# ChenAnno/FashionERN_AAAI2024

Hardware: AMD Instinct MI355X
Metric: composed queries/sec (higher is better)
Workload: dtype f32; 1 GPU; FashionIQ ViT-B/16 composed queries: 64-query batch per GPU vs 46k-image fused gallery (BASELINE.json configs[1]); clip=ViT-B-16, query_batch_per_gpu=64, gallery_rows=46000, gallery_dtype=f32, feature_dim=512, top_k=50, batches_in_flight=4, hw_queues=4, parallelism=dp1 queries

## Files before the change

### fashionern_aaai2024_amd/csrc/api.hip

```cpp
#include <hip/hip_runtime.h>

#include <algorithm>
#include <cmath>
#include <cstdio>
#include <cstdlib>
#include <cstring>
#include <map>
#include <string>
#include <vector>

#include "../../include/fern.h"
#include "kernels.h"
#include "live.h"

using namespace fern;

static thread_local std::string g_last_error;

static int fail(int code, const std::string& msg) {
    g_last_error = msg;
    return code;
}
#define HIP_TRY(expr)                                                                                   \
    do {                                                                                                \
// ... 310 lines not shown
    FERN_TRY(prof_open(c, PROF_GEMM, 2.0 * p1.M * (double)p1.N * p1.K + 2.0 * p2.M * (double)p2.N * p2.K, s, &slot, p1.M, p1.N, p1.K, 350 + p1.epi));
    const hipError_t le = launch_gemm_mxbf_pair(p1, p2, s);
    HIP_TRY_PROF(le, c, slot);
    if (slot >= 0) {
        c->recs[slot].dispatches = gemm_last_dispatches();
        c->recs[slot].extra_flops = 2.0 * p2.M * (double)p2.N * p2.K;
    }
    return prof_close(c, slot, s);
}
static int run_attention(fern_ctx* c, const AttnParams& a, hipStream_t s) {
    int slot;
    FERN_TRY(prof_open(c, PROF_ATTN, 4.0 * a.batch * a.heads * (double)a.s_q * a.s_k * a.hd, s, &slot, a.batch * a.heads, a.s_q, a.hd, a.causal));
    const hipError_t le = launch_attention(a, s);
    HIP_TRY_PROF(le, c, slot);
    return prof_close(c, slot, s);
}

static int make_bf16(fern_ctx* c, LinearW* L);

static int upload(fern_ctx* c, const float* h, size_t n, const float** out) {
    float* d = nullptr;
    HIP_TRY(hipMalloc(&d, std::max<size_t>(n, 4) * sizeof(float)));
    HIP_TRY(hipMemcpy(d, h, n * sizeof(float), hipMemcpyHostToDevice));
    c->owned[c->cur_group].push_back(d);
    *out = d;
    return FERN_OK;
}
static int need(fern_ctx* c, const std::string& key, std::vector<int64_t> shape, const HostTensor** out) {
    auto it = c->host.find(key);
    if (it == c->host.end()) return fail(FERN_ERR_STATE, "missing weight: " + key);
// ... 808 lines not shown
    const fern_clip_config& cf = W.cfg;
    const int g = cf.image_size / cf.patch_size;
    if (text) *T = Tower{W.tblocks.data(), batch, cf.context_length, cf.t_width, cf.t_heads, cf.t_mlp, 1};
    else *T = Tower{W.vblocks.data(), batch, g * g + 1, cf.v_width, cf.v_heads, cf.v_mlp, 0};
    tower_forms(c, text, T);
    const size_t R = (size_t)T->R();
    FERN_TRY(ws_get(c, R * T->width, &T->X));
    FERN_TRY(ws_get(c, R * T->width, &T->XN));
    FERN_TRY(ws_get(c, R * 3 * T->width, &T->QKV));
    FERN_TRY(ws_get(c, R * T->width, &T->ATT));
    return ws_get(c, R * T->mlp, &T->H);
}

static int run_gemm_form(fern_ctx* c, Form f, const GemmParams& p, hipStream_t s) { return f == F32 ? run_gemm(c, p, s) : run_gemm_b(c, p, s); }

static int ln_gemm(const Tower& T, Form f, const LNW& ln, const LinearW& L, void* C, long ldc, int epi, bool out_bf16, hipStream_t s, GemmParams* p) {
    const long R = T.R();
    const int w = T.width;
    switch (f) {
    case F32:
        HIP_TRY(launch_layernorm(T.X, nullptr, ln.g, ln.b, T.XN, R, w, w, w, 1e-5f, s));
        *p = gemm_desc(T.XN, w, L, reinterpret_cast<float*>(C), ldc, (int)R, epi);
        break;
    case BF16:
        HIP_TRY(launch_layernorm_bf16(T.X, ln.g, ln.b, T.XNb(), R, w, w, w, 1e-5f, s));
        *p = gemm_desc_b(T.XNb(), w, L, C, ldc, (int)R, epi, out_bf16);
        break;
    case FP8:
        HIP_TRY(launch_layernorm_fp8(T.X, ln.g, ln.b, T.XN8(), T.SA(), R, w, w, w, 1e-5f, s));
        *p = gemm_desc_f8(T.XN8(), T.SA(), w, L, C, ldc, (int)R, epi, out_bf16);
        break;
    case MX:
        HIP_TRY(launch_layernorm_mx8(T.Xb ? nullptr : T.X, ln.g, ln.b, T.XN8(), T.SM(), R, R, w, w, w, 1e-5f, s, T.Xb));
        *p = gemm_desc_mx(T.XN8(), T.SM(), R, w, L, C, ldc, (int)R, epi, out_bf16);
        break;
    }
    return FERN_OK;
}
static void residual_in_place(const Tower& T, GemmParams* p) {
    if (T.Xb) p->Rb = T.Xb;
    else p->R = T.X;
}

static int prep_qkv(fern_ctx*, const Tower& T, const ClipBlockW& Bk, hipStream_t s, GemmParams* p) {
    return ln_gemm(T, T.attn, Bk.ln1, Bk.qkv, T.QKV, 3 * T.width, EPI_BIAS, true, s, p);
}
static int prep_out(fern_ctx* c, const Tower& T, const ClipBlockW& Bk, hipStream_t s, GemmParams* p) {
    const long R = T.R();
    const int w = T.width, hd = w / T.heads;
    const bool fused = T.attn == MX && hd % 32 == 0;
    if (T.attn == F32) {
        AttnParams a{T.QKV, T.QKV + w, T.QKV + 2 * w, T.ATT, 3L * w, 3L * w, 3L * w, (long)w,
                     T.batch, T.heads, hd, T.S, T.S, T.causal, 1.0f / std::sqrt((float)hd)};
        FERN_TRY(run_attention(c, a, s));
    } else {
        AttnParams a{nullptr, nullptr, nullptr, nullptr, 3L * w, 3L * w, 3L * w, (long)w,
                     T.batch, T.heads, hd, T.S, T.S, T.causal, 1.0f / std::sqrt((float)hd), T.ATTb(), T.QKVb(), T.QKVb() + w, T.QKVb() + 2 * w};
        if (fused) { a.out_b = nullptr; a.out_q8 = T.ATT8(); a.out_scales = T.SM(); a.out_srows = R; }
        FERN_TRY(run_attention(c, a, s));
    }
    switch (T.attn) {
    case F32: *p = gemm_desc(T.ATT, w, Bk.out, T.X, w, (int)R, EPI_BIAS_RESIDUAL); break;
    case BF16: *p = gemm_desc_b(T.ATTb(), w, Bk.out, T.X, w, (int)R, EPI_BIAS_RESIDUAL, false); break;
    case FP8:
        HIP_TRY(launch_quantize_rows_fp8(T.ATTb(), nullptr, w, T.ATT8(), w, T.SA(), R, w, s));
        *p = gemm_desc_f8(T.ATT8(), T.SA(), w, Bk.out, T.X, w, (int)R, EPI_BIAS_RESIDUAL, false);
        break;
    case MX:
        if (!fused) HIP_TRY(launch_quantize_mx8(T.ATTb(), nullptr, w, T.ATT8(), w, T.SM(), R, R, w, s));
        *p = gemm_desc_mx(T.ATT8(), T.SM(), R, w, Bk.out, T.stream(), w, (int)R, EPI_BIAS_RESIDUAL, T.Xb != nullptr);
        break;
    }
    residual_in_place(T, p);
    return FERN_OK;
}
static int prep_fc(fern_ctx* c, const Tower& T, const ClipBlockW& Bk, hipStream_t s, GemmParams* p) {
    FERN_TRY(ln_gemm(T, T.mlpf, Bk.ln2, Bk.fc, T.H, T.mlp, clip_mlp_epi(c), T.mlpf != MX, s, p));
    if (T.mlpf == MX) { p->out_mx8 = 1; p->mxc = T.SH(); p->mxc_rows = T.R(); }
    return FERN_OK;
}
static int prep_proj(fern_ctx*, const Tower& T, const ClipBlockW& Bk, hipStream_t s, GemmParams* p) {
    const long R = T.R();
    const int w = T.width, mlp = T.mlp;
    switch (T.mlpf) {
    case F32: *p = gemm_desc(T.H, mlp, Bk.proj, T.X, w, (int)R, EPI_BIAS_RESIDUAL); break;
    case BF16: *p = gemm_desc_b(T.Hb(), mlp, Bk.proj, T.X, w, (int)R, EPI_BIAS_RESIDUAL, false); break;
    case FP8:
        HIP_TRY(launch_quantize_rows_fp8(T.Hb(), nullptr, mlp, T.H8(FP8), mlp, T.SA(), R, mlp, s));
        *p = gemm_desc_f8(T.H8(FP8), T.SA(), mlp, Bk.proj, T.X, w, (int)R, EPI_BIAS_RESIDUAL, false);
        break;
    case MX:
        *p = gemm_desc_mx(T.H8(MX), T.SH(), R, mlp, Bk.proj, T.stream(), w, (int)R, EPI_BIAS_RESIDUAL, T.Xb != nullptr);
        break;
// ... 271 lines not shown
    const fern_clip_config& cf = W.cfg;
    Tower V, T;
    float* CLS;
    int* eot;
    FERN_TRY(tower_open(c, false, b, &V));
    FERN_TRY(ws_get(c, (size_t)b * V.width, &CLS));
    FERN_TRY(tower_open(c, true, b, &T));
    FERN_TRY(ws_get(c, (size_t)b, &eot));
    FERN_TRY(vit_front(c, images, V.X, V.H, b, s));
    HIP_TRY(launch_layernorm(V.X, nullptr, W.ln_pre.g, W.ln_pre.b, V.X, V.R(), V.width, V.width, V.width, 1e-5f, s));
    HIP_TRY(launch_text_embed(tokens, W.tok_emb, W.tpos, T.X, eot, b, T.S, T.width, cf.vocab_size, c->tok_flag, s));
    const int vfull = cf.v_layers - 1;
    const int paired = vfull < cf.t_layers ? vfull : cf.t_layers;
    const bool mx = V.attn == MX;
    auto run_pair = [&](const GemmParams& pv, const GemmParams& pt) { return mx ? run_gemm_b_pair(c, pv, pt, s) : run_gemm_pair(c, pv, pt, s); };
    for (int l = 0; l < paired; ++l) {
        const ClipBlockW &Bv = V.blocks[l], &Bt = T.blocks[l];
        GemmParams pv, pt;
        FERN_TRY(prep_qkv(c, V, Bv, s, &pv));
        FERN_TRY(prep_qkv(c, T, Bt, s, &pt));
        FERN_TRY(run_pair(pv, pt));
        FERN_TRY(prep_out(c, V, Bv, s, &pv));
        FERN_TRY(prep_out(c, T, Bt, s, &pt));
        FERN_TRY(run_pair(pv, pt));
        FERN_TRY(prep_fc(c, V, Bv, s, &pv));
        FERN_TRY(prep_fc(c, T, Bt, s, &pt));
        FERN_TRY(run_pair(pv, pt));
        FERN_TRY(prep_proj(c, V, Bv, s, &pv));
        FERN_TRY(prep_proj(c, T, Bt, s, &pt));
        FERN_TRY(run_pair(pv, pt));
    }
    for (int l = paired; l < vfull; ++l) FERN_TRY(tower_block(c, V, l, s));
    for (int l = paired; l < cf.t_layers; ++l) FERN_TRY(tower_block(c, T, l, s));
    FERN_TRY(vit_tail(c, V, CLS, out_img, s));
    return text_tail(c, T.X, T.XN, eot, out_global, out_seq, b, s);
}

static int check_token_flag(fern_ctx* c, const char* fn) {
    if (!c->tok_flag) return FERN_OK;
    const int v = __atomic_load_n(c->tok_flag, __ATOMIC_RELAXED);
    if (v == 0) return FERN_OK;
    __atomic_store_n(c->tok_flag, 0, __ATOMIC_RELAXED);
// ... 1129 lines not shown
```

### fashionern_aaai2024_amd/csrc/attn.hip

```cpp
#include "kernels.h"

#include <cstdlib>

namespace fern {

typedef float f32x16 __attribute__((ext_vector_type(16)));
typedef float f32x4 __attribute__((ext_vector_type(4)));
typedef short bf16x8 __attribute__((ext_vector_type(8)));
typedef short s16x4 __attribute__((ext_vector_type(4)));
typedef unsigned u32x4_t __attribute__((ext_vector_type(4)));

extern __shared__ __attribute__((aligned(16))) char attn_smem[];

struct LanePos { int l31, lh, tr_off; };
__device__ __forceinline__ LanePos lane_pos() {
    const int lane = threadIdx.x & 63, lh = lane >> 5;
    return {lane & 31, lh, ((lane & 15) >> 2) * 64 + (((lane >> 4) & 1) * 16 + (lane & 3) * 4) * 2 + lh * 4 * 64};
}

template <int HDP_>
struct F32Form {
    static constexpr int HDP = HDP_;
    static constexpr bool BF16 = false;
    static constexpr int KS = HDP + 4;
// ... 246 lines not shown
__device__ __forceinline__ void store_out(const f32x16 (&o)[F::HDP / 32], float inv, int b, int h, int qi, int lh, const AttnParams& p) {
    if constexpr (!F::BF16) store_f32(o, inv, b, h, qi, lh, p);
    else if (p.out_q8) store_mx(o, inv, b, h, qi, lh, p);
    else store_bf16(o, inv, b, h, qi, lh, p);
}

template <int NB>
__device__ __forceinline__ void zero_acc(f32x16 (&o)[NB]) {
#pragma unroll
    for (int db = 0; db < NB; ++db)
#pragma unroll
        for (int r = 0; r < 16; ++r) o[db][r] = 0.0f;
}

template <class F, int NT, bool CAUSAL, int NW>
__device__ __forceinline__ void resident_walk(const AttnParams& p) {
    constexpr int ROWS = NT * 32;
    const int wave = threadIdx.x >> 6;
    const int b = blockIdx.x / p.heads, h = blockIdx.x % p.heads;
    F::template stage<ROWS>(p, b, h, 0, ROWS, threadIdx.x, NW * 64);
    __syncthreads();
    const LanePos lp = lane_pos();

    const int nqt = (p.s_q + 31) / 32;
    for (int qt = wave; qt < nqt; qt += NW) {
        const int qi = qt * 32 + lp.l31;
        typename F::Q qf;
        F::load_q(qf, p, b, h, qi < p.s_q ? qi : p.s_q - 1, lp.lh, true);
        f32x16 o[F::HDP / 32];
        zero_acc(o);
        float m = -INFINITY, sum = 0.0f;
        const int nt = CAUSAL ? (qt + 1 < NT ? qt + 1 : NT) : NT;
#pragma unroll 1
        for (int t = 0; t < nt; ++t) F::template key_tile<CAUSAL, ROWS>(t, t, qi, lp, p, qf, m, sum, o);
// ... 22 lines not shown
        const int nt = nkt - t0 < CT ? nkt - t0 : CT;
        if (t0) __syncthreads();
        F::template stage<ROWS>(p, b, h, t0 * 32, whole_image ? ROWS : nt * 32, threadIdx.x, stride);
        __syncthreads();
        if (!active) continue;
#pragma unroll 1
        for (int t = 0; t < nt; ++t) F::template key_tile<false, ROWS>(t, t0 + t, qi, lp, p, qf, m, sum, o);
    }
    if (!active) return;
    sum += __shfl_xor(sum, 32);
    store_out<F>(o, 1.0f / sum, b, h, qi, lp.lh, p);
}

template <int HDP, int NT, bool CAUSAL, int NW>
__global__ __launch_bounds__(NW * 64) void attn_f32_kernel(AttnParams p) {
    resident_walk<F32Form<HDP>, NT, CAUSAL, NW>(p);
}

template <int HDP, int NT, bool CAUSAL, int NW>
__global__ __launch_bounds__(NW * 64) void attn_bf16_kernel(AttnParams p) {
    resident_walk<Bf16Form<HDP>, NT, CAUSAL, NW>(p);
}

template <int HDP, int NT, int NW, int KH>
__global__ __launch_bounds__(NW * 64, 2) void attn_f32_chunked_kernel(AttnParams p) {
    chunk_walk<F32Form<HDP>, (NT + KH - 1) / KH>(p, StreamGroup{(int)blockIdx.x, 0, (p.s_q + 31) / 32}, NT, NW * 64, true);
}

constexpr int STREAM_CT = 4;
constexpr int STREAM_MAX_WAVES = 8;

__device__ __forceinline__ StreamGroup stream_group(int s_q) {
    const int nqt = (s_q + 31) / 32, ng = (nqt + STREAM_MAX_WAVES - 1) / STREAM_MAX_WAVES;
    const int base = nqt / ng, rem = nqt % ng, grp = blockIdx.x % ng;
    return {(int)(blockIdx.x / ng), grp * base + (grp < rem ? grp : rem), base + (grp < rem ? 1 : 0)};
}

template <int HDP>
__global__ __launch_bounds__(STREAM_MAX_WAVES * 64, HDP <= 64 ? 4 : 2) void attn_f32_stream_kernel(AttnParams p) {
    chunk_walk<F32Form<HDP>, STREAM_CT>(p, stream_group(p.s_q), (p.s_k + 31) / 32, blockDim.x, false);
}

template <int HDP>
__global__ __launch_bounds__(STREAM_MAX_WAVES * 64, 4) void attn_bf16_stream_kernel(AttnParams p) {
    chunk_walk<Bf16Form<HDP>, STREAM_CT>(p, stream_group(p.s_q), (p.s_k + 31) / 32, blockDim.x, false);
}

template <auto Kern>
static hipError_t launch_kernel(const AttnParams& p, dim3 grid, dim3 block, size_t lds, hipStream_t s) {
    static bool attr_set = false;
    if (!attr_set && lds > 48 * 1024) {
        hipError_t e = hipFuncSetAttribute(reinterpret_cast<const void*>(Kern), hipFuncAttributeMaxDynamicSharedMemorySize, (int)lds);
        if (e != hipSuccess) return e;
        attr_set = true;
    }
    FERN_LAUNCH(Kern, grid, block, lds, s, p);
    return hipGetLastError();
}

template <class F, int NT, bool CAUSAL>
// ... 102 lines not shown
        for (int u = 0; u < UNR; ++u) {
            const int j = j0 + 4 * u;
            vv[u] = vb[(long)(j < p.s_k ? j : p.s_k - 1) * p.ldv];
        }
#pragma unroll
        for (int u = 0; u < UNR; ++u) {
            const int j = j0 + 4 * u;
            acc = __builtin_fmaf(j < p.s_k ? sc[j] : 0.0f, vv[u], acc);
        }
    }
    red[wave][lane] = acc;
    __syncthreads();
    if (wave == 0 && lane < hd)
        p.out[(long)b * p.ldo + (long)h * hd + lane] = (((red[0][lane] + red[1][lane]) + red[2][lane]) + red[3][lane]) * (1.0f / sum);
}
hipError_t launch_attention(const AttnParams& p, hipStream_t s) {
    if (p.batch <= 0 || p.heads <= 0 || p.s_q <= 0 || p.s_k <= 0 || p.s_k > ATTN_MAX_KEYS) return hipErrorInvalidValue;
    if (p.causal && p.s_q != p.s_k) return hipErrorInvalidValue;
    if (p.qb || p.kb || p.vb) {
        if (!p.qb || !p.kb || !p.vb || (!p.out_b && !p.out_q8) || (p.out_q8 && (!p.out_scales || (p.hd & 31))) || (p.hd & 7) || (p.ldq & 7) || (p.ldk & 7) || (p.ldv & 7) || (p.ldo & 3)) return hipErrorInvalidValue;
        return launch_hd<Bf16Form>(p, s);
    }
    if (p.out_b || p.out_q8) return hipErrorInvalidValue;
    if ((p.hd & 3) || (p.ldq & 3) || (p.ldk & 3) || (p.ldv & 3) || (p.ldo & 3)) return hipErrorInvalidValue;
    if (p.s_q == 1 && !p.causal && p.hd <= 64 && p.s_k <= SQ1_MAX_KEYS) {
        FERN_LAUNCH(attn_f32_single_query_kernel<25>, dim3(p.batch * p.heads), dim3(256), 0, s, p);
        return hipGetLastError();
    }
    return launch_hd<F32Form>(p, s);
}

}
```

### fashionern_aaai2024_amd/csrc/elem.hip

```cpp
#include "kernels.h"
#include "row_ops.h"
#include <type_traits>

namespace fern {

__device__ __forceinline__ float wave_max(float v) {
    v = fmaxf(v, dpp_move<0xB1>(v));
    v = fmaxf(v, dpp_move<0x4E>(v));
    v = fmaxf(v, dpp_move<0x141>(v));
    v = fmaxf(v, dpp_move<0x140>(v));
    return fmaxf(fmaxf(lane_f(v, 0), lane_f(v, 16)), fmaxf(lane_f(v, 32), lane_f(v, 48)));
}
__device__ __forceinline__ float quad_max(float v) {
    v = fmaxf(v, dpp_move<0xB1>(v));
    return fmaxf(v, dpp_move<0x4E>(v));
}
__device__ __forceinline__ float oct_max(float v) { v = quad_max(v); return fmaxf(v, dpp_move<0x141>(v)); }

template <class V>
constexpr int chunk_width = sizeof(V) / sizeof(float);

__device__ __forceinline__ void load8(float (&v)[8], const float* p) {
    const f32x4 a = load4(p), b = load4(p + 4);
#pragma unroll
// ... 128 lines not shown
            if ((i * 64 + lane) * 4 < d) am = chunk_amax(am, r.v[i]);
        row_store_fp8(r.v, am, y + row * ldy, scale + row, d, lane);
    }
};
struct RowToMx8 {
    unsigned char* y; long ldy; unsigned char* scales; long srows;
    __device__ void operator()(const RowRegs& r, long row, int d, int lane) const {
#pragma unroll
        for (int i = 0; i < MAXV; ++i) {
            const int c = (i * 64 + lane) * 4;
            store_mx8(r.v[i], c < d, y + row * ldy, c, scales, srows, row, lane);
        }
    }
};
template <class T, class Out>
__global__ __launch_bounds__(256) void layernorm_kernel(const T* x, const float* gamma, const float* beta, Out out, long rows, int d, long ldx,
                                                        float eps, const float* res) {
    const long row = (long)blockIdx.x * ROWS_PER_BLOCK + (threadIdx.x >> 6);
    const int lane = threadIdx.x & 63;
    if (row >= rows) return;
    RowRegs r;
    row_load(r, x + row * ldx, d, lane);
    if constexpr (std::is_same_v<Out, RowToF32>) {
        if (res) {
            RowRegs q;
            row_load(q, res + row * ldx, d, lane);
#pragma unroll
            for (int i = 0; i < MAXV; ++i) r.v[i] += q.v[i];
        }
    }
    row_layernorm(r, gamma, beta, d, lane, eps);
    out(r, row, d, lane);
}

__device__ __forceinline__ void row_load8(float (&v)[8], const unsigned short* xb, const float* xf, long at, bool live) {
#pragma unroll
    for (int e = 0; e < 8; ++e) v[e] = 0.f;
    if (live) {
        if (xb) load8(v, xb + at);
        else load8(v, xf + at);
    }
}
__global__ __launch_bounds__(256) void quantize_rows_fp8_kernel(const unsigned short* xb, const float* xf, long ldx, unsigned char* y, long ldy,
                                                                float* scale, long rows, int d) {
    const long row = (long)blockIdx.x * ROWS_PER_BLOCK + (threadIdx.x >> 6);
    const int lane = threadIdx.x & 63;
    if (row >= rows) return;
    float v[8][8];
// ... 19 lines not shown
        store_mx8(v, c < d, y + row * ldy, c, scales, srows, row, lane);
    }
}

template <class F>
static void with_nv(int d, F f) {
    switch (d / 256) {
        case 1: f(std::integral_constant<int, 1>{}); break;
        case 2: f(std::integral_constant<int, 2>{}); break;
        case 3: f(std::integral_constant<int, 3>{}); break;
        default: f(std::integral_constant<int, 4>{}); break;
    }
}

template <int NV, int RPW>
__global__ __launch_bounds__(256) void layernorm_rows_kernel(const float* x, const float* gamma, const float* beta, float* y, long rows, long ldx,
                                                             long ldy, float eps) {
    constexpr int D = 256 * NV;
    const int lane = threadIdx.x & 63;
    const long row0 = ((long)blockIdx.x * ROWS_PER_BLOCK + (threadIdx.x >> 6)) * RPW;
    if (row0 >= rows) return;
    f32x4 v[RPW][NV];
#pragma unroll
    for (int r = 0; r < RPW; ++r) {
        const long row = row0 + r < rows ? row0 + r : rows - 1;
#pragma unroll
        for (int i = 0; i < NV; ++i) v[r][i] = load4(x + row * ldx + (i * 64 + lane) * 4);
    }
    f32x4 g[NV], bb[NV];
#pragma unroll
    for (int i = 0; i < NV; ++i) {
        g[i] = load4(gamma + (i * 64 + lane) * 4);
        bb[i] = load4(beta + (i * 64 + lane) * 4);
    }
    float mean[RPW], rstd[RPW];
// ... 8 lines not shown
            for (int e = 0; e < 4; ++e) { const float t = v[r][i][e] - mean[r]; q += t * t; }
        rstd[r] = rsqrtf(wave_sum(q) / (float)D + eps);
    }
#pragma unroll
    for (int r = 0; r < RPW; ++r) {
        const long row = row0 + r;
#pragma unroll
        for (int i = 0; i < NV; ++i) {
            f32x4 o;
#pragma unroll
            for (int e = 0; e < 4; ++e) o[e] = ln_affine(v[r][i][e], mean[r], rstd[r], g[i][e], bb[i][e]);
            if (row < rows) *reinterpret_cast<f32x4*>(y + row * ldy + (i * 64 + lane) * 4) = o;
        }
    }
}
constexpr int LN_RPW = 4;
static bool launch_ln_rows(const float* x, const float* gamma, const float* beta, float* y, long rows, int d, long ldx, long ldy, float eps,
                           hipStream_t s) {
    if (d % 256 || d > 1024) return false;
    if (((uintptr_t)gamma & 15) || ((uintptr_t)beta & 15)) return false;
    const dim3 grid((unsigned)((rows + ROWS_PER_BLOCK * LN_RPW - 1) / (ROWS_PER_BLOCK * LN_RPW)));
    with_nv(d, [&](auto nv) {
        hipLaunchKernelGGL((layernorm_rows_kernel<decltype(nv)::value, LN_RPW>), grid, dim3(256), 0, s, x, gamma, beta, y, rows, ldx, ldy, eps);
    });
    return true;
}

template <int NV, class T>
__global__ __launch_bounds__(256) void layernorm_half_kernel(const T* x, const float* gamma, const float* beta, unsigned char* y, unsigned char* scales,
                                                             long srows, long rows, long ldx, long ldy, float eps) {
    constexpr int D = 256 * NV;
    const int lane = threadIdx.x & 63, l31 = lane & 31, lh = lane >> 5;
    const long rowp = ((long)blockIdx.x * ROWS_PER_BLOCK + (threadIdx.x >> 6)) * 2;
    if (rowp >= rows) return;
    const long row = rowp + lh;
    const long rrow = row < rows ? row : rows - 1;
    float v[NV][8], g[NV][8], bb[NV][8];
#pragma unroll
    for (int i = 0; i < NV; ++i) load8(v[i], x + rrow * ldx + (i * 32 + l31) * 8);
#pragma unroll
    for (int i = 0; i < NV; ++i) {
        load8(g[i], gamma + (i * 32 + l31) * 8);
        load8(bb[i], beta + (i * 32 + l31) * 8);
    }
    const auto half_sum = [&](float t) {
        t += dpp_move<0xB1>(t);
        t += dpp_move<0x4E>(t);
        t += dpp_move<0x141>(t);
        t += dpp_move<0x140>(t);
        const float lo = lane_f(t, 0) + lane_f(t, 16), hi = lane_f(t, 32) + lane_f(t, 48);
        return lh ? hi : lo;
    };
    const float mean = ln_mean(v, half_sum, (float)D);
    const float rstd = ln_rstd(v, mean, [](int) { return true; }, half_sum, (float)D, eps);
#pragma unroll
    for (int i = 0; i < NV; ++i) {
        float o[8];
#pragma unroll
        for (int e = 0; e < 8; ++e) o[e] = ln_affine(v[i][e], mean, rstd, g[i][e], bb[i][e]);
        store_mx8<true>(o, row < rows, y + row * ldy, (i * 32 + l31) * 8, scales, srows, row, lane);
    }
}
template <class T>
static bool launch_ln_half(const T* x, const float* gamma, const float* beta, unsigned char* y, unsigned char* scales, long srows, long rows, int d,
                           long ldx, long ldy, float eps, hipStream_t s) {
    if (d % 256 || d > 1024 || (ldx & 7) || (ldy & 7) || ((uintptr_t)x & 15) || ((uintptr_t)y & 7) || ((uintptr_t)gamma & 15) || ((uintptr_t)beta & 15)) return false;
    const dim3 grid((unsigned)((rows + ROWS_PER_BLOCK * 2 - 1) / (ROWS_PER_BLOCK * 2)));
    with_nv(d, [&](auto nv) {
        hipLaunchKernelGGL((layernorm_half_kernel<decltype(nv)::value, T>), grid, dim3(256), 0, s, x, gamma, beta, y, scales, srows, rows, ldx, ldy, eps);
    });
    return true;
}

struct PatchRow {
    const float* src;
    int img, patch, pp;
    __device__ const float* at(int k) const {
        const int ch = k / pp, rem = k % pp;
        return src + ((long)ch * img + rem / patch) * img + rem % patch;
    }
};
__device__ __forceinline__ PatchRow patch_row(const float* images, long row, int img, int patch, int grid) {
// ... 433 lines not shown
                                long ldx, long ldy, float eps, hipStream_t s) {
    if (rows <= 0) return hipSuccess;
    if (bad_width(d) || (ldx & 3) || (ldy & 3)) return hipErrorInvalidValue;
    return launch_ln_row(x, nullptr, gamma, beta, RowToFp8{y, ldy, scale}, rows, d, ldx, eps, s);
}
hipError_t launch_layernorm_mx8(const float* x, const float* gamma, const float* beta, unsigned char* y, unsigned char* scales, long srows,
                                long rows, int d, long ldx, long ldy, float eps, hipStream_t s, const unsigned short* x_bf16) {
    if (rows <= 0) return hipSuccess;
    if (d <= 0 || d % 128 || d > 256 * MAXV || (ldx & 3) || (ldy & 3) || srows < rows) return hipErrorInvalidValue;
    if (x_bf16 ? launch_ln_half(x_bf16, gamma, beta, y, scales, srows, rows, d, ldx, ldy, eps, s)
               : launch_ln_half(x, gamma, beta, y, scales, srows, rows, d, ldx, ldy, eps, s))
        return hipGetLastError();
    const RowToMx8 out{y, ldy, scales, srows};
    return x_bf16 ? launch_ln_row(x_bf16, nullptr, gamma, beta, out, rows, d, ldx, eps, s) : launch_ln_row(x, nullptr, gamma, beta, out, rows, d, ldx, eps, s);
}
hipError_t launch_im2col_mx8(const float* images, unsigned char* y, unsigned char* scales, long srows, int b, int img, int patch, int grid,
                             hipStream_t s) {
    const long rows = (long)b * grid * grid;
    if (rows <= 0) return hipSuccess;
    const int d = 3 * patch * patch;
    if (d % 128 || d > 256 * MAXV || (patch & 3) || (img & 3) || grid * patch != img || srows < rows) return hipErrorInvalidValue;
    hipLaunchKernelGGL(im2col_mx8_kernel, row_grid(rows), dim3(256), 0, s, images, y, scales, srows, rows, img, patch, grid);
    return hipGetLastError();
}
hipError_t launch_im2col_bf16(const float* images, unsigned short* y, int b, int img, int patch, int grid, hipStream_t s) {
    const long rows = (long)b * grid * grid;
    if (rows <= 0) return hipSuccess;
    const int d = 3 * patch * patch;
    if (d % 32 || d > 256 * MAXV || (patch & 3) || (img & 3) || grid * patch != img) return hipErrorInvalidValue;
    hipLaunchKernelGGL(im2col_bf16_kernel, row_grid(rows), dim3(256), 0, s, images, y, rows, img, patch, grid);
// ... 170 lines not shown
```

### fashionern_aaai2024_amd/csrc/kernels.h

```cpp
#pragma once
#include <hip/hip_runtime.h>
#include <stdint.h>

#include <string>

#ifdef __HIPCC__
#include <hip/hip_ext.h>
#endif
#include <vector>

namespace fern {

struct LaunchTimer {
    std::vector<hipEvent_t> events;
    std::vector<hipEvent_t>* pool;
};
extern thread_local LaunchTimer* g_launch_timer;
struct LaunchTimerPause {
    LaunchTimer* saved;
    LaunchTimerPause() : saved(g_launch_timer) { g_launch_timer = nullptr; }
    ~LaunchTimerPause() { g_launch_timer = saved; }
};
hipEvent_t launch_timer_event();
#ifdef __HIPCC__
// ... 201 lines not shown
struct AttnParams {
    const float* q; const float* k; const float* v; float* out;
    long ldq, ldk, ldv, ldo;
    int batch, heads, hd, s_q, s_k, causal;
    float scale;
    unsigned short* out_b;
    const unsigned short* qb;
    const unsigned short* kb;
    const unsigned short* vb;
    unsigned char* out_q8;
    unsigned char* out_scales;
    long out_srows;
};
constexpr int ATTN_MAX_KEYS = 4096;
hipError_t launch_attention(const AttnParams& p, hipStream_t s);

hipError_t launch_layernorm(const float* x, const float* res, const float* gamma, const float* beta, float* y,
                            long rows, int d, long ldx, long ldy, float eps, hipStream_t s);
hipError_t launch_layernorm_bf16(const float* x, const float* gamma, const float* beta, unsigned short* y, long rows, int d, long ldx,
                                 long ldy, float eps, hipStream_t s);
hipError_t launch_layernorm_fp8(const float* x, const float* gamma, const float* beta, unsigned char* y, float* scale, long rows, int d,
                                long ldx, long ldy, float eps, hipStream_t s);
hipError_t launch_quantize_rows_fp8(const unsigned short* x_bf16, const float* x_f32, long ldx, unsigned char* y, long ldy, float* scale,
                                    long rows, int d, hipStream_t s);
hipError_t launch_layernorm_mx8(const float* x, const float* gamma, const float* beta, unsigned char* y, unsigned char* scales, long srows,
                                long rows, int d, long ldx, long ldy, float eps, hipStream_t s, const unsigned short* x_bf16 = nullptr );
hipError_t launch_quantize_mx8(const unsigned short* x_bf16, const float* x_f32, long ldx, unsigned char* y, long ldy, unsigned char* scales,
                               long srows, long rows, int d, hipStream_t s);
hipError_t launch_im2col_bf16(const float* images, unsigned short* y, int b, int img, int patch, int grid, hipStream_t s);
hipError_t launch_patch_rows_f32(const float* images, float* y, int b, int img, int patch, int grid, int kp, hipStream_t s);
hipError_t launch_im2col_mx8(const float* images, unsigned char* y, unsigned char* scales, long srows, int b, int img, int patch, int grid,
                             hipStream_t s);
hipError_t launch_l2norm(const float* x, long ldx, float* y, long ldy, long rows, int d, float eps, int mode, hipStream_t s,
                         const float* x2 = nullptr);
hipError_t launch_mean_rows(const float* x, long ldx, float* y, long ldy, long n, int P, int d, long group_stride, long row_add,
                            hipStream_t s);
hipError_t launch_ce_diag_mean(const float* logits, long ld, int n, float scale, float* row_loss, float* out, hipStream_t s);
hipError_t launch_gather_rows(const float* x, long ldx, float* y, long ldy, long n, int d, int group, long group_stride, long row_add,
                              const int* idx, hipStream_t s);
hipError_t launch_gather_rows_bf16(const unsigned short* x, long ldx, float* y, long ldy, long n, int d, long row_stride, hipStream_t s);
hipError_t launch_bert_embed(const float* cls, const float* local, const float* seq, const float* type_emb,
// ... 92 lines not shown
```

Baseline: 2953 queries/sec.

## Co-launch image and text tower layernorm and attention as paired kernels

```diff
diff --git a/fashionern_aaai2024_amd/csrc/api.hip b/fashionern_aaai2024_amd/csrc/api.hip
--- a/fashionern_aaai2024_amd/csrc/api.hip
+++ b/fashionern_aaai2024_amd/csrc/api.hip
@@ -348,6 +348,26 @@
     const hipError_t le = launch_attention(a, s);
     HIP_TRY_PROF(le, c, slot);
     return prof_close(c, slot, s);
+}
+static int run_attention_pair(fern_ctx* c, const AttnParams& a, const AttnParams& t, hipStream_t s) {
+    int slot;
+    const double work = 4.0 * a.batch * a.heads * (double)a.s_q * a.s_k * a.hd + 4.0 * t.batch * t.heads * (double)t.s_q * t.s_k * t.hd;
+    FERN_TRY(prof_open(c, PROF_ATTN, work, s, &slot, a.batch * a.heads, a.s_q, a.hd, a.causal));
+    const hipError_t le = launch_attention_pair(a, t, s);
+    HIP_TRY_PROF(le, c, slot);
+    return prof_close(c, slot, s);
+}
+enum { STAGE_PAIR_LN = 1, STAGE_PAIR_ATTN = 2 };
+static int stage_pairs() {
+    static const int on = [] {
+        const char* e = getenv("FERN_STAGE_PAIR");
+        if (!e) return STAGE_PAIR_LN | STAGE_PAIR_ATTN;
+        if (e[0] == '0') return 0;
+        if (!strcmp(e, "ln")) return (int)STAGE_PAIR_LN;
+        if (!strcmp(e, "attn")) return (int)STAGE_PAIR_ATTN;
+        return STAGE_PAIR_LN | STAGE_PAIR_ATTN;
+    }();
+    return on;
 }
 
 static int make_bf16(fern_ctx* c, LinearW* L);
@@ -1186,27 +1206,41 @@
 
 static int run_gemm_form(fern_ctx* c, Form f, const GemmParams& p, hipStream_t s) { return f == F32 ? run_gemm(c, p, s) : run_gemm_b(c, p, s); }
 
-static int ln_gemm(const Tower& T, Form f, const LNW& ln, const LinearW& L, void* C, long ldc, int epi, bool out_bf16, hipStream_t s, GemmParams* p) {
+static int ln_launch(const Tower& T, Form f, const LNW& ln, hipStream_t s) {
     const long R = T.R();
     const int w = T.width;
     switch (f) {
-    case F32:
-        HIP_TRY(launch_layernorm(T.X, nullptr, ln.g, ln.b, T.XN, R, w, w, w, 1e-5f, s));
-        *p = gemm_desc(T.XN, w, L, reinterpret_cast<float*>(C), ldc, (int)R, epi);
-        break;
-    case BF16:
-        HIP_TRY(launch_layernorm_bf16(T.X, ln.g, ln.b, T.XNb(), R, w, w, w, 1e-5f, s));
-        *p = gemm_desc_b(T.XNb(), w, L, C, ldc, (int)R, epi, out_bf16);
-        break;
-    case FP8:
-        HIP_TRY(launch_layernorm_fp8(T.X, ln.g, ln.b, T.XN8(), T.SA(), R, w, w, w, 1e-5f, s));
-        *p = gemm_desc_f8(T.XN8(), T.SA(), w, L, C, ldc, (int)R, epi, out_bf16);
-        break;
-    case MX:
-        HIP_TRY(launch_layernorm_mx8(T.Xb ? nullptr : T.X, ln.g, ln.b, T.XN8(), T.SM(), R, R, w, w, w, 1e-5f, s, T.Xb));
-        *p = gemm_desc_mx(T.XN8(), T.SM(), R, w, L, C, ldc, (int)R, epi, out_bf16);
-        break;
-    }
+    case F32: HIP_TRY(launch_layernorm(T.X, nullptr, ln.g, ln.b, T.XN, R, w, w, w, 1e-5f, s)); break;
+    case BF16: HIP_TRY(launch_layernorm_bf16(T.X, ln.g, ln.b, T.XNb(), R, w, w, w, 1e-5f, s)); break;
+    case FP8: HIP_TRY(launch_layernorm_fp8(T.X, ln.g, ln.b, T.XN8(), T.SA(), R, w, w, w, 1e-5f, s)); break;
+    case MX: HIP_TRY(launch_layernorm_mx8(T.Xb ? nullptr : T.X, ln.g, ln.b, T.XN8(), T.SM(), R, R, w, w, w, 1e-5f, s, T.Xb)); break;
+    }
+    return FERN_OK;
+}
+static bool ln_side(const Tower& T, Form f, const LNW& ln, LnSide* o) {
+    const long R = T.R();
+    const int w = T.width;
+    *o = LnSide{T.X, ln.g, ln.b, R, w, w, w, 1e-5f};
+    switch (f) {
+    case F32: o->y = T.XN; return true;
+    case BF16: o->yb = T.XNb(); return true;
+    case MX: o->y8 = T.XN8(); o->scales = T.SM(); o->srows = R; return !T.Xb;
+    default: return false;
+    }
+}
+static GemmParams ln_gemm_desc(const Tower& T, Form f, const LinearW& L, void* C, long ldc, int epi, bool out_bf16) {
+    const long R = T.R();
+    const int w = T.width;
+    switch (f) {
+    case F32: return gemm_desc(T.XN, w, L, reinterpret_cast<float*>(C), ldc, (int)R, epi);
+    case BF16: return gemm_desc_b(T.XNb(), w, L, C, ldc, (int)R, epi, out_bf16);
+    case FP8: return gemm_desc_f8(T.XN8(), T.SA(), w, L, C, ldc, (int)R, epi, out_bf16);
+    default: return gemm_desc_mx(T.XN8(), T.SM(), R, w, L, C, ldc, (int)R, epi, out_bf16);
+    }
+}
+static int ln_gemm(const Tower& T, Form f, const LNW& ln, const LinearW& L, void* C, long ldc, int epi, bool out_bf16, hipStream_t s, GemmParams* p) {
+    FERN_TRY(ln_launch(T, f, ln, s));
+    *p = ln_gemm_desc(T, f, L, C, ldc, epi, out_bf16);
     return FERN_OK;
 }
 static void residual_in_place(const Tower& T, GemmParams* p) {
@@ -1214,23 +1248,27 @@
     else p->R = T.X;
 }
 
+static GemmParams desc_qkv(const Tower& T, const ClipBlockW& Bk) { return ln_gemm_desc(T, T.attn, Bk.qkv, T.QKV, 3 * T.width, EPI_BIAS, true); }
 static int prep_qkv(fern_ctx*, const Tower& T, const ClipBlockW& Bk, hipStream_t s, GemmParams* p) {
-    return ln_gemm(T, T.attn, Bk.ln1, Bk.qkv, T.QKV, 3 * T.width, EPI_BIAS, true, s, p);
-}
-static int prep_out(fern_ctx* c, const Tower& T, const ClipBlockW& Bk, hipStream_t s, GemmParams* p) {
+    FERN_TRY(ln_launch(T, T.attn, Bk.ln1, s));
+    *p = desc_qkv(T, Bk);
+    return FERN_OK;
+}
+static bool attn_quantises(const Tower& T) { return T.attn == MX && (T.width / T.heads) % 32 == 0; }
+static AttnParams attn_desc(const Tower& T) {
+    const int w = T.width, hd = w / T.heads;
+    if (T.attn == F32)
+        return AttnParams{T.QKV, T.QKV + w, T.QKV + 2 * w, T.ATT, 3L * w, 3L * w, 3L * w, (long)w,
+                          T.batch, T.heads, hd, T.S, T.S, T.causal, 1.0f / std::sqrt((float)hd)};
+    AttnParams a{nullptr, nullptr, nullptr, nullptr, 3L * w, 3L * w, 3L * w, (long)w,
+                 T.batch, T.heads, hd, T.S, T.S, T.causal, 1.0f / std::sqrt((float)hd), T.ATTb(), T.QKVb(), T.QKVb() + w, T.QKVb() + 2 * w};
+    if (attn_quantises(T)) { a.out_b = nullptr; a.out_q8 = T.ATT8(); a.out_scales = T.SM(); a.out_srows = T.R(); }
+    return a;
+}
+static int desc_out(const Tower& T, const ClipBlockW& Bk, hipStream_t s, GemmParams* p) {
     const long R = T.R();
-    const int w = T.width, hd = w / T.heads;
-    const bool fused = T.attn == MX && hd % 32 == 0;
-    if (T.attn == F32) {
-        AttnParams a{T.QKV, T.QKV + w, T.QKV + 2 * w, T.ATT, 3L * w, 3L * w, 3L * w, (long)w,
-                     T.batch, T.heads, hd, T.S, T.S, T.causal, 1.0f / std::sqrt((float)hd)};
-        FERN_TRY(run_attention(c, a, s));
-    } else {
-        AttnParams a{nullptr, nullptr, nullptr, nullptr, 3L * w, 3L * w, 3L * w, (long)w,
-                     T.batch, T.heads, hd, T.S, T.S, T.causal, 1.0f / std::sqrt((float)hd), T.ATTb(), T.QKVb(), T.QKVb() + w, T.QKVb() + 2 * w};
-        if (fused) { a.out_b = nullptr; a.out_q8 = T.ATT8(); a.out_scales = T.SM(); a.out_srows = R; }
-        FERN_TRY(run_attention(c, a, s));
-    }
+    const int w = T.width;
+    const bool fused = attn_quantises(T);
     switch (T.attn) {
     case F32: *p = gemm_desc(T.ATT, w, Bk.out, T.X, w, (int)R, EPI_BIAS_RESIDUAL); break;
     case BF16: *p = gemm_desc_b(T.ATTb(), w, Bk.out, T.X, w, (int)R, EPI_BIAS_RESIDUAL, false); break;
@@ -1246,9 +1284,18 @@
     residual_in_place(T, p);
     return FERN_OK;
 }
+static int prep_out(fern_ctx* c, const Tower& T, const ClipBlockW& Bk, hipStream_t s, GemmParams* p) {
+    FERN_TRY(run_attention(c, attn_desc(T), s));
+    return desc_out(T, Bk, s, p);
+}
+static GemmParams desc_fc(fern_ctx* c, const Tower& T, const ClipBlockW& Bk) {
+    GemmParams p = ln_gemm_desc(T, T.mlpf, Bk.fc, T.H, T.mlp, clip_mlp_epi(c), T.mlpf != MX);
+    if (T.mlpf == MX) { p.out_mx8 = 1; p.mxc = T.SH(); p.mxc_rows = T.R(); }
+    return p;
+}
 static int prep_fc(fern_ctx* c, const Tower& T, const ClipBlockW& Bk, hipStream_t s, GemmParams* p) {
-    FERN_TRY(ln_gemm(T, T.mlpf, Bk.ln2, Bk.fc, T.H, T.mlp, clip_mlp_epi(c), T.mlpf != MX, s, p));
-    if (T.mlpf == MX) { p->out_mx8 = 1; p->mxc = T.SH(); p->mxc_rows = T.R(); }
+    FERN_TRY(ln_launch(T, T.mlpf, Bk.ln2, s));
+    *p = desc_fc(c, T, Bk);
     return FERN_OK;
 }
 static int prep_proj(fern_ctx*, const Tower& T, const ClipBlockW& Bk, hipStream_t s, GemmParams* p) {
@@ -1550,18 +1597,32 @@
     const int paired = vfull < cf.t_layers ? vfull : cf.t_layers;
     const bool mx = V.attn == MX;
     auto run_pair = [&](const GemmParams& pv, const GemmParams& pt) { return mx ? run_gemm_b_pair(c, pv, pt, s) : run_gemm_pair(c, pv, pt, s); };
+    const int stages = stage_pairs();
+    auto ln_pair = [&](Form fv, const LNW& lv, Form ft, const LNW& lt) -> int {
+        LnSide sv, st;
+        if ((stages & STAGE_PAIR_LN) && ln_side(V, fv, lv, &sv) && ln_side(T, ft, lt, &st)) {
+            HIP_TRY(launch_layernorm_pair(sv, st, s));
+            return FERN_OK;
+        }
+        FERN_TRY(ln_launch(V, fv, lv, s));
+        return ln_launch(T, ft, lt, s);
+    };
     for (int l = 0; l < paired; ++l) {
         const ClipBlockW &Bv = V.blocks[l], &Bt = T.blocks[l];
         GemmParams pv, pt;
-        FERN_TRY(prep_qkv(c, V, Bv, s, &pv));
-        FERN_TRY(prep_qkv(c, T, Bt, s, &pt));
+        FERN_TRY(ln_pair(V.attn, Bv.ln1, T.attn, Bt.ln1));
+        FERN_TRY(run_pair(desc_qkv(V, Bv), desc_qkv(T, Bt)));
+        if (stages & STAGE_PAIR_ATTN) {
+            FERN_TRY(run_attention_pair(c, attn_desc(V), attn_desc(T), s));
+        } else {
+            FERN_TRY(run_attention(c, attn_desc(V), s));
+            FERN_TRY(run_attention(c, attn_desc(T), s));
+        }
+        FERN_TRY(desc_out(V, Bv, s, &pv));
+        FERN_TRY(desc_out(T, Bt, s, &pt));
         FERN_TRY(run_pair(pv, pt));
-        FERN_TRY(prep_out(c, V, Bv, s, &pv));
-        FERN_TRY(prep_out(c, T, Bt, s, &pt));
-        FERN_TRY(run_pair(pv, pt));
-        FERN_TRY(prep_fc(c, V, Bv, s, &pv));
-        FERN_TRY(prep_fc(c, T, Bt, s, &pt));
-        FERN_TRY(run_pair(pv, pt));
+        FERN_TRY(ln_pair(V.mlpf, Bv.ln2, T.mlpf, Bt.ln2));
+        FERN_TRY(run_pair(desc_fc(c, V, Bv), desc_fc(c, T, Bt)));
         FERN_TRY(prep_proj(c, V, Bv, s, &pv));
         FERN_TRY(prep_proj(c, T, Bt, s, &pt));
         FERN_TRY(run_pair(pv, pt));
diff --git a/fashionern_aaai2024_amd/csrc/attn.hip b/fashionern_aaai2024_amd/csrc/attn.hip
--- a/fashionern_aaai2024_amd/csrc/attn.hip
+++ b/fashionern_aaai2024_amd/csrc/attn.hip
@@ -284,10 +284,10 @@
 }
 
 template <class F, int NT, bool CAUSAL, int NW>
-__device__ __forceinline__ void resident_walk(const AttnParams& p) {
+__device__ __forceinline__ void resident_walk(const AttnParams& p, const int bh) {
     constexpr int ROWS = NT * 32;
     const int wave = threadIdx.x >> 6;
-    const int b = blockIdx.x / p.heads, h = blockIdx.x % p.heads;
+    const int b = bh / p.heads, h = bh % p.heads;
     F::template stage<ROWS>(p, b, h, 0, ROWS, threadIdx.x, NW * 64);
     __syncthreads();
     const LanePos lp = lane_pos();
@@ -340,12 +340,12 @@
 
 template <int HDP, int NT, bool CAUSAL, int NW>
 __global__ __launch_bounds__(NW * 64) void attn_f32_kernel(AttnParams p) {
-    resident_walk<F32Form<HDP>, NT, CAUSAL, NW>(p);
+    resident_walk<F32Form<HDP>, NT, CAUSAL, NW>(p, blockIdx.x);
 }
 
 template <int HDP, int NT, bool CAUSAL, int NW>
 __global__ __launch_bounds__(NW * 64) void attn_bf16_kernel(AttnParams p) {
-    resident_walk<Bf16Form<HDP>, NT, CAUSAL, NW>(p);
+    resident_walk<Bf16Form<HDP>, NT, CAUSAL, NW>(p, blockIdx.x);
 }
 
 template <int HDP, int NT, int NW, int KH>
@@ -370,6 +370,17 @@
 template <int HDP>
 __global__ __launch_bounds__(STREAM_MAX_WAVES * 64, 4) void attn_bf16_stream_kernel(AttnParams p) {
     chunk_walk<Bf16Form<HDP>, STREAM_CT>(p, stream_group(p.s_q), (p.s_k + 31) / 32, blockDim.x, false);
+}
+
+template <int HDP>
+__global__ __launch_bounds__(8 * 64, 2) void attn_f32_pair_kernel(AttnParams pi, AttnParams pt, int ni) {
+    if ((int)blockIdx.x < ni) chunk_walk<F32Form<HDP>, 4>(pi, StreamGroup{(int)blockIdx.x, 0, (pi.s_q + 31) / 32}, 7, 8 * 64, true);
+    else resident_walk<F32Form<HDP>, 3, true, 8>(pt, (int)blockIdx.x - ni);
+}
+template <int HDP>
+__global__ __launch_bounds__(8 * 64, 2) void attn_bf16_pair_kernel(AttnParams pi, AttnParams pt, int ni) {
+    if ((int)blockIdx.x < ni) resident_walk<Bf16Form<HDP>, 7, false, 8>(pi, blockIdx.x);
+    else resident_walk<Bf16Form<HDP>, 3, true, 8>(pt, (int)blockIdx.x - ni);
 }
 
 template <auto Kern>
@@ -502,15 +513,23 @@
     if (wave == 0 && lane < hd)
         p.out[(long)b * p.ldo + (long)h * hd + lane] = (((red[0][lane] + red[1][lane]) + red[2][lane]) + red[3][lane]) * (1.0f / sum);
 }
-hipError_t launch_attention(const AttnParams& p, hipStream_t s) {
+static hipError_t attn_params_check(const AttnParams& p, bool* bf16) {
     if (p.batch <= 0 || p.heads <= 0 || p.s_q <= 0 || p.s_k <= 0 || p.s_k > ATTN_MAX_KEYS) return hipErrorInvalidValue;
     if (p.causal && p.s_q != p.s_k) return hipErrorInvalidValue;
-    if (p.qb || p.kb || p.vb) {
+    *bf16 = p.qb || p.kb || p.vb;
+    if (*bf16) {
         if (!p.qb || !p.kb || !p.vb || (!p.out_b && !p.out_q8) || (p.out_q8 && (!p.out_scales || (p.hd & 31))) || (p.hd & 7) || (p.ldq & 7) || (p.ldk & 7) || (p.ldv & 7) || (p.ldo & 3)) return hipErrorInvalidValue;
-        return launch_hd<Bf16Form>(p, s);
+        return hipSuccess;
     }
     if (p.out_b || p.out_q8) return hipErrorInvalidValue;
     if ((p.hd & 3) || (p.ldq & 3) || (p.ldk & 3) || (p.ldv & 3) || (p.ldo & 3)) return hipErrorInvalidValue;
+    return hipSuccess;
+}
+hipError_t launch_attention(const AttnParams& p, hipStream_t s) {
+    bool bf16;
+    const hipError_t ce = attn_params_check(p, &bf16);
+    if (ce != hipSuccess) return ce;
+    if (bf16) return launch_hd<Bf16Form>(p, s);
     if (p.s_q == 1 && !p.causal && p.hd <= 64 && p.s_k <= SQ1_MAX_KEYS) {
         FERN_LAUNCH(attn_f32_single_query_kernel<25>, dim3(p.batch * p.heads), dim3(256), 0, s, p);
         return hipGetLastError();
@@ -518,4 +537,31 @@
     return launch_hd<F32Form>(p, s);
 }
 
-}
+template <auto Kern>
+static hipError_t launch_pair_kernel(const AttnParams& pi, const AttnParams& pt, size_t lds, hipStream_t s) {
+    static bool attr_set = false;
+    if (!attr_set) {
+        hipError_t e = hipFuncSetAttribute(reinterpret_cast<const void*>(Kern), hipFuncAttributeMaxDynamicSharedMemorySize, (int)lds);
+        if (e != hipSuccess) return e;
+        attr_set = true;
+    }
+    const int ni = pi.batch * pi.heads;
+    FERN_LAUNCH(Kern, dim3(ni + pt.batch * pt.heads), dim3(8 * 64), lds, s, pi, pt, ni);
+    return hipGetLastError();
+}
+hipError_t launch_attention_pair(const AttnParams& pi, const AttnParams& pt, hipStream_t s) {
+    bool bi, bt;
+    hipError_t e = attn_params_check(pi, &bi);
+    if (e == hipSuccess) e = attn_params_check(pt, &bt);
+    if (e != hipSuccess) return e;
+    const int nti = (pi.s_k + 31) / 32, ntt = (pt.s_k + 31) / 32;
+    const bool shapes = bi == bt && !pi.causal && pt.causal && pi.hd > 32 && pi.hd <= 64 && pt.hd > 32 && pt.hd <= 64 && nti > 4 && nti <= 7 &&
+                        ntt > 1 && ntt <= 3 && pi.s_q > 1 && !stream_forced() && (bi || (chunked_allowed() && pi.s_q <= 256));
+    if (!shapes) {
+        e = launch_attention(pi, s);
+        return e != hipSuccess ? e : launch_attention(pt, s);
+    }
+    if (bi) return launch_pair_kernel<attn_bf16_pair_kernel<64>>(pi, pt, Bf16Form<64>::image_bytes(7 * 32), s);
+    return launch_pair_kernel<attn_f32_pair_kernel<64>>(pi, pt, F32Form<64>::image_bytes(4 * 32), s);
+}
+}
diff --git a/fashionern_aaai2024_amd/csrc/elem.hip b/fashionern_aaai2024_amd/csrc/elem.hip
--- a/fashionern_aaai2024_amd/csrc/elem.hip
+++ b/fashionern_aaai2024_amd/csrc/elem.hip
@@ -166,9 +166,9 @@
     }
 };
 template <class T, class Out>
-__global__ __launch_bounds__(256) void layernorm_kernel(const T* x, const float* gamma, const float* beta, Out out, long rows, int d, long ldx,
-                                                        float eps, const float* res) {
-    const long row = (long)blockIdx.x * ROWS_PER_BLOCK + (threadIdx.x >> 6);
+__device__ __forceinline__ void layernorm_body(long blk, const T* x, const float* gamma, const float* beta, Out out, long rows, int d, long ldx,
+                                               float eps, const float* res) {
+    const long row = blk * ROWS_PER_BLOCK + (threadIdx.x >> 6);
     const int lane = threadIdx.x & 63;
     if (row >= rows) return;
     RowRegs r;
@@ -184,6 +184,11 @@
     row_layernorm(r, gamma, beta, d, lane, eps);
     out(r, row, d, lane);
 }
+template <class T, class Out>
+__global__ __launch_bounds__(256) void layernorm_kernel(const T* x, const float* gamma, const float* beta, Out out, long rows, int d, long ldx,
+                                                        float eps, const float* res) {
+    layernorm_body(blockIdx.x, x, gamma, beta, out, rows, d, ldx, eps, res);
+}
 
 __device__ __forceinline__ void row_load8(float (&v)[8], const unsigned short* xb, const float* xf, long at, bool live) {
 #pragma unroll
@@ -233,11 +238,11 @@
 }
 
 template <int NV, int RPW>
-__global__ __launch_bounds__(256) void layernorm_rows_kernel(const float* x, const float* gamma, const float* beta, float* y, long rows, long ldx,
-                                                             long ldy, float eps) {
+__device__ __forceinline__ void layernorm_rows_body(long blk, const float* x, const float* gamma, const float* beta, float* y, long rows, long ldx,
+                                                    long ldy, float eps) {
     constexpr int D = 256 * NV;
     const int lane = threadIdx.x & 63;
-    const long row0 = ((long)blockIdx.x * ROWS_PER_BLOCK + (threadIdx.x >> 6)) * RPW;
+    const long row0 = (blk * ROWS_PER_BLOCK + (threadIdx.x >> 6)) * RPW;
     if (row0 >= rows) return;
     f32x4 v[RPW][NV];
 #pragma unroll
@@ -276,12 +281,21 @@
         }
     }
 }
+template <int NV, int RPW>
+__global__ __launch_bounds__(256) void layernorm_rows_kernel(const float* x, const float* gamma, const float* beta, float* y, long rows, long ldx,
+                                                             long ldy, float eps) {
+    layernorm_rows_body<NV, RPW>(blockIdx.x, x, gamma, beta, y, rows, ldx, ldy, eps);
+}
 constexpr int LN_RPW = 4;
+static bool ln_rows_ok(const float* gamma, const float* beta, int d) {
+    if (d % 256 || d > 1024) return false;
+    return !(((uintptr_t)gamma & 15) || ((uintptr_t)beta & 15));
+}
+static unsigned ln_rows_blocks(long rows) { return (unsigned)((rows + ROWS_PER_BLOCK * LN_RPW - 1) / (ROWS_PER_BLOCK * LN_RPW)); }
 static bool launch_ln_rows(const float* x, const float* gamma, const float* beta, float* y, long rows, int d, long ldx, long ldy, float eps,
                            hipStream_t s) {
-    if (d % 256 || d > 1024) return false;
-    if (((uintptr_t)gamma & 15) || ((uintptr_t)beta & 15)) return false;
-    const dim3 grid((unsigned)((rows + ROWS_PER_BLOCK * LN_RPW - 1) / (ROWS_PER_BLOCK * LN_RPW)));
+    if (!ln_rows_ok(gamma, beta, d)) return false;
+    const dim3 grid(ln_rows_blocks(rows));
     with_nv(d, [&](auto nv) {
         hipLaunchKernelGGL((layernorm_rows_kernel<decltype(nv)::value, LN_RPW>), grid, dim3(256), 0, s, x, gamma, beta, y, rows, ldx, ldy, eps);
     });
@@ -289,11 +303,11 @@
 }
 
 template <int NV, class T>
-__global__ __launch_bounds__(256) void layernorm_half_kernel(const T* x, const float* gamma, const float* beta, unsigned char* y, unsigned char* scales,
-                                                             long srows, long rows, long ldx, long ldy, float eps) {
+__device__ __forceinline__ void layernorm_half_body(long blk, const T* x, const float* gamma, const float* beta, unsigned char* y, unsigned char* scales,
+                                                    long srows, long rows, long ldx, long ldy, float eps) {
     constexpr int D = 256 * NV;
     const int lane = threadIdx.x & 63, l31 = lane & 31, lh = lane >> 5;
-    const long rowp = ((long)blockIdx.x * ROWS_PER_BLOCK + (threadIdx.x >> 6)) * 2;
+    const long rowp = (blk * ROWS_PER_BLOCK + (threadIdx.x >> 6)) * 2;
     if (rowp >= rows) return;
     const long row = rowp + lh;
     const long rrow = row < rows ? row : rows - 1;
@@ -323,11 +337,20 @@
         store_mx8<true>(o, row < rows, y + row * ldy, (i * 32 + l31) * 8, scales, srows, row, lane);
     }
 }
+template <int NV, class T>
+__global__ __launch_bounds__(256) void layernorm_half_kernel(const T* x, const float* gamma, const float* beta, unsigned char* y, unsigned char* scales,
+                                                             long srows, long rows, long ldx, long ldy, float eps) {
+    layernorm_half_body<NV, T>(blockIdx.x, x, gamma, beta, y, scales, srows, rows, ldx, ldy, eps);
+}
+static bool ln_half_ok(const void* x, const float* gamma, const float* beta, const unsigned char* y, int d, long ldx, long ldy) {
+    return !(d % 256 || d > 1024 || (ldx & 7) || (ldy & 7) || ((uintptr_t)x & 15) || ((uintptr_t)y & 7) || ((uintptr_t)gamma & 15) || ((uintptr_t)beta & 15));
+}
+static unsigned ln_half_blocks(long rows) { return (unsigned)((rows + ROWS_PER_BLOCK * 2 - 1) / (ROWS_PER_BLOCK * 2)); }
 template <class T>
 static bool launch_ln_half(const T* x, const float* gamma, const float* beta, unsigned char* y, unsigned char* scales, long srows, long rows, int d,
                            long ldx, long ldy, float eps, hipStream_t s) {
-    if (d % 256 || d > 1024 || (ldx & 7) || (ldy & 7) || ((uintptr_t)x & 15) || ((uintptr_t)y & 7) || ((uintptr_t)gamma & 15) || ((uintptr_t)beta & 15)) return false;
-    const dim3 grid((unsigned)((rows + ROWS_PER_BLOCK * 2 - 1) / (ROWS_PER_BLOCK * 2)));
+    if (!ln_half_ok(x, gamma, beta, y, d, ldx, ldy)) return false;
+    const dim3 grid(ln_half_blocks(rows));
     with_nv(d, [&](auto nv) {
         hipLaunchKernelGGL((layernorm_half_kernel<decltype(nv)::value, T>), grid, dim3(256), 0, s, x, gamma, beta, y, scales, srows, rows, ldx, ldy, eps);
     });
@@ -791,6 +814,45 @@
     const RowToMx8 out{y, ldy, scales, srows};
     return x_bf16 ? launch_ln_row(x_bf16, nullptr, gamma, beta, out, rows, d, ldx, eps, s) : launch_ln_row(x, nullptr, gamma, beta, out, rows, d, ldx, eps, s);
 }
+template <int NVA, int NVB>
+__global__ __launch_bounds__(256) void layernorm_rows_pair_kernel(LnSide a, LnSide b, unsigned na) {
+    if (blockIdx.x < na) layernorm_rows_body<NVA, LN_RPW>(blockIdx.x, a.x, a.gamma, a.beta, a.y, a.rows, a.ldx, a.ldy, a.eps);
+    else layernorm_rows_body<NVB, LN_RPW>(blockIdx.x - na, b.x, b.gamma, b.beta, b.y, b.rows, b.ldx, b.ldy, b.eps);
+}
+template <int NVA>
+__global__ __launch_bounds__(256) void layernorm_half_bf16_pair_kernel(LnSide a, LnSide b, unsigned na) {
+    if (blockIdx.x < na) layernorm_half_body<NVA, float>(blockIdx.x, a.x, a.gamma, a.beta, a.y8, a.scales, a.srows, a.rows, a.ldx, a.ldy, a.eps);
+    else layernorm_body<float, RowToBf16>(blockIdx.x - na, b.x, b.gamma, b.beta, RowToBf16{b.yb, b.ldy}, b.rows, b.d, b.ldx, b.eps, nullptr);
+}
+static hipError_t launch_ln_side(const LnSide& p, hipStream_t s) {
+    if (p.y) return launch_layernorm(p.x, nullptr, p.gamma, p.beta, p.y, p.rows, p.d, p.ldx, p.ldy, p.eps, s);
+    if (p.yb) return launch_layernorm_bf16(p.x, p.gamma, p.beta, p.yb, p.rows, p.d, p.ldx, p.ldy, p.eps, s);
+    if (p.y8) return launch_layernorm_mx8(p.x, p.gamma, p.beta, p.y8, p.scales, p.srows, p.rows, p.d, p.ldx, p.ldy, p.eps, s);
+    return hipErrorInvalidValue;
+}
+hipError_t launch_layernorm_pair(const LnSide& a, const LnSide& b, hipStream_t s) {
+    const auto sides_valid = [](const LnSide& p) { return !(bad_width(p.d) || (p.ldx & 3) || (p.ldy & 3)); };
+    if (a.rows > 0 && b.rows > 0 && sides_valid(a) && sides_valid(b)) {
+        if (a.y && b.y && ln_rows_ok(a.gamma, a.beta, a.d) && ln_rows_ok(b.gamma, b.beta, b.d)) {
+            const unsigned na = ln_rows_blocks(a.rows), nb = ln_rows_blocks(b.rows);
+            with_nv(a.d, [&](auto nva) {
+                with_nv(b.d, [&](auto nvb) {
+                    hipLaunchKernelGGL((layernorm_rows_pair_kernel<decltype(nva)::value, decltype(nvb)::value>), dim3(na + nb), dim3(256), 0, s, a, b, na);
+                });
+            });
+            return hipGetLastError();
+        }
+        if (a.y8 && b.yb && a.d % 128 == 0 && a.srows >= a.rows && ln_half_ok(a.x, a.gamma, a.beta, a.y8, a.d, a.ldx, a.ldy)) {
+            const unsigned na = ln_half_blocks(a.rows), nb = row_grid(b.rows).x;
+            with_nv(a.d, [&](auto nva) {
+                hipLaunchKernelGGL((layernorm_half_bf16_pair_kernel<decltype(nva)::value>), dim3(na + nb), dim3(256), 0, s, a, b, na);
+            });
+            return hipGetLastError();
+        }
+    }
+    const hipError_t e = launch_ln_side(a, s);
+    return e != hipSuccess ? e : launch_ln_side(b, s);
+}
 hipError_t launch_im2col_mx8(const float* images, unsigned char* y, unsigned char* scales, long srows, int b, int img, int patch, int grid,
                              hipStream_t s) {
     const long rows = (long)b * grid * grid;
diff --git a/fashionern_aaai2024_amd/csrc/kernels.h b/fashionern_aaai2024_amd/csrc/kernels.h
--- a/fashionern_aaai2024_amd/csrc/kernels.h
+++ b/fashionern_aaai2024_amd/csrc/kernels.h
@@ -239,6 +239,7 @@
 };
 constexpr int ATTN_MAX_KEYS = 4096;
 hipError_t launch_attention(const AttnParams& p, hipStream_t s);
+hipError_t launch_attention_pair(const AttnParams& image, const AttnParams& text, hipStream_t s);
 
 hipError_t launch_layernorm(const float* x, const float* res, const float* gamma, const float* beta, float* y,
                             long rows, int d, long ldx, long ldy, float eps, hipStream_t s);
@@ -250,6 +251,12 @@
                                     long rows, int d, hipStream_t s);
 hipError_t launch_layernorm_mx8(const float* x, const float* gamma, const float* beta, unsigned char* y, unsigned char* scales, long srows,
                                 long rows, int d, long ldx, long ldy, float eps, hipStream_t s, const unsigned short* x_bf16 = nullptr );
+struct LnSide {
+    const float* x; const float* gamma; const float* beta;
+    long rows; int d; long ldx, ldy; float eps;
+    float* y; unsigned short* yb; unsigned char* y8; unsigned char* scales; long srows;
+};
+hipError_t launch_layernorm_pair(const LnSide& image, const LnSide& text, hipStream_t s);
 hipError_t launch_quantize_mx8(const unsigned short* x_bf16, const float* x_f32, long ldx, unsigned char* y, long ldy, unsigned char* scales,
                                long srows, long rows, int d, hipStream_t s);
 hipError_t launch_im2col_bf16(const float* images, unsigned short* y, int b, int img, int patch, int grid, hipStream_t s);
```

New measurement: 2970 queries/sec (median of 6 runs). About the same (+0.6%).
